# raguilar011095/planet_heightmap_generation

Measured on AMD Instinct MI355X. Metric: Mcells·iter/s, terrain-post erosion stack, higher is better.
Workload: dtype f64

## Files before the change

planet_heightmap_generation_amd/csrc/device.h:

```cpp
#pragma once
#include <hip/hip_runtime.h>

#include <cstdint>
#include <cstdio>
#include <map>
#include <string>
#include <vector>

#include "host_util.h"

#include "erode_ops.h"
#include "flood_ops.h"
#include "wo_internal.h"

namespace wo {

struct HipError { std::string msg; };

#define WO_HIP(call)                                                                                   \
    do {                                                                                               \
        hipError_t e_ = (call);                                                                        \
        if (e_ != hipSuccess)                                                                          \
            throw ::wo::HipError{std::string(#call) + " -> " + hipGetErrorString(e_) + " (" + __FILE__ + ":" + \
                                 std::to_string(__LINE__) + ")"};                                      \
// ... 77 lines not shown
    int32_t* h_count = nullptr;
    float* d_redoE = nullptr; int32_t* d_pendingEver = nullptr; int64_t redoCalls = 0;
    unsigned long long *h_word = nullptr, *d_word = nullptr; uint32_t wordSerial = 0;
    wo::FloodScratch flood;
    wo::FloodExchange floodX;
    void* floodLink = nullptr; void (*floodLinkFree)(void*) = nullptr;
    wo_flood_gpu fgpu;

    int32_t *d_off = nullptr, *d_adj = nullptr;
    float *d_dist = nullptr, *d_xyz = nullptr;
    float *d_e = nullptr, *d_e2 = nullptr, *d_hot = nullptr, *d_orig = nullptr;
    uint8_t *d_ocean = nullptr, *d_coast = nullptr;
    int64_t mirrorMaskVersion = -1;
    uint8_t* d_oceanKnown = nullptr; int32_t* d_maskDiff = nullptr; bool oceanKnownValid = false;
    bool hot_valid = false;
    float* d_savedE = nullptr; uint8_t* d_savedOcean = nullptr; bool saved = false;
    uint8_t* d_tables = nullptr;
    bool scratch = false;
    bool landIdentity = false;
    int64_t floodPrefixMirror = -1, floodPrefixStatic = -1;
    bool floodPrefixOk = false;
    int32_t *d_landIdx = nullptr, *d_land[2] = {nullptr, nullptr}, *d_rank = nullptr;
    int32_t* d_landInit = nullptr; int64_t oceanVersion = 0, landListsOcean = -1; bool landListsMirror = false; int32_t landListsL = -1;
    uint32_t* d_keys[2] = {nullptr, nullptr};
    float *d_cellDist = nullptr, *d_flow = nullptr;
    wo::SolveTask* d_task = nullptr; wo::SolveOut* d_out = nullptr; int32_t *d_haloSend = nullptr, *d_haloRecv = nullptr; float *d_haloBuf = nullptr, *h_haloBuf = nullptr; int32_t nHaloSend = 0, nHaloRecv = 0;
    int32_t* d_flowCnt = nullptr; wo::TargetRank* d_tr = nullptr; wo::EventList* d_ev = nullptr; float* d_me = nullptr;
    int32_t *d_carveSlot = nullptr, *d_carveDeps = nullptr, *d_carveDepCnt = nullptr, *d_carveDepPos = nullptr; uint32_t* d_rs[2] = {nullptr, nullptr}; int rsFlip[2] = {0, 0};    wo::CarveRec* d_carveRecs = nullptr; wo::CarveExpect* d_carveExpect = nullptr; unsigned long long* d_carveG = nullptr;    int32_t* d_carveSlotDone = nullptr; int64_t carveCap = 0;
    unsigned long long* d_accCnt = nullptr;
    int32_t *d_ftLr = nullptr, *d_ftParent = nullptr, *d_ftExtCnt = nullptr; uint32_t* d_ftInflow = nullptr; unsigned long long* d_ftRootAcc = nullptr;
    int32_t *d_jump = nullptr, *d_nj = nullptr;
    int32_t* d_doneAt = nullptr;
    double* d_totalExcess = nullptr;
    float *d_glac = nullptr, *d_iceFlow = nullptr;
    int32_t *d_iceTarget = nullptr, *d_arank = nullptr;
    uint8_t* d_iceUp = nullptr;
    int32_t *d_patchOrder = nullptr, *d_slotOf = nullptr, *d_patchPending = nullptr, *d_patchTotals = nullptr, *d_patchBlk = nullptr; int64_t patchVersion = -1; bool patchMirror = false; int32_t numPatches = 0; int64_t lastPatchLaunches = 1; int64_t solveCalls = 0;
    hipStream_t side = nullptr; hipEvent_t evFork = nullptr, evJoin = nullptr; bool onSide = false;
    uint32_t* d_basinKey = nullptr; int32_t* d_basinVals[2] = {nullptr, nullptr}; int32_t *d_basinJ = nullptr, *d_basinSlot = nullptr, *d_basinRange = nullptr; uint8_t* d_basinLong = nullptr; int64_t basinLaunches = 0; wo::Affine* d_affine[2] = {nullptr, nullptr};    int64_t solvePassSerial = 0;
    int32_t* h_patchTotals = nullptr;
    int32_t *d_listA = nullptr, *d_listB = nullptr, *d_counters = nullptr;
    void* d_sortTemp = nullptr; size_t sortTempBytes = 0;
    int landCur = 0;
    int32_t L = 0;

    struct Import {
        uint8_t* img = nullptr; int64_t imgCap = 0;
        int32_t* label = nullptr;
        uint8_t* flags = nullptr;
        int32_t* lists = nullptr;
        uint8_t* seedOcean = nullptr;
        int32_t* blockCounts = nullptr;
        int32_t* totals = nullptr; int32_t* h_totals = nullptr;
    } imp;

    struct Mirror {
        bool built = false, active = false;
        int32_t *perm = nullptr, *inv = nullptr, *off = nullptr, *adj = nullptr;
        float *dist = nullptr, *xyz = nullptr, *e = nullptr, *e2 = nullptr, *hot = nullptr;
        uint8_t *ocean = nullptr, *coast = nullptr;
        wo::hvec<int32_t> h_perm, h_morton;
        wo::hvec<uint8_t> h_mask;
        int64_t version = 0;
        int32_t *o_off = nullptr, *o_adj = nullptr; float *o_dist = nullptr, *o_xyz = nullptr, *o_e = nullptr, *o_e2 = nullptr;
        uint8_t *o_ocean = nullptr, *o_coast = nullptr;
    } mirror;
// ... 67 lines not shown
```

planet_heightmap_generation_amd/csrc/erode_ops.h:

```cpp
#pragma once
#include <cmath>
#include <cstdint>
#include <cstring>

#include "noise.h"

namespace wo {

constexpr int WO_MAX_DEG = 24;
constexpr int32_t WO_NOT_DONE = 0x7fffffff;

#ifndef WO_TASK_ALIGN
#define WO_TASK_ALIGN 16
#endif
struct alignas(WO_TASK_ALIGN) SolveTask {
    int32_t predSelf, predT, predT2;
    uint32_t flags;
    float e0r, e0t, e0t2;
    float cellDistT;
    double factor;
    int32_t pad_[2];
};
static_assert(sizeof(SolveTask) == 48, "one 48-byte record per task");
#ifndef WO_PATCH_CELLS
// ... 597 lines not shown
        const double h = masked(r);
        int32_t b, nbs[WO_ROW];
        const int deg = load_row(F, r, b, nbs);
        if (deg <= WO_ROW) {
            float mh[WO_ROW], dd[WO_ROW];
#pragma unroll
            for (int k = 0; k < WO_ROW; ++k) mh[k] = masked(nbs[k]);
            load_row_dist(F, b, deg, dd);
#pragma unroll
            for (int k = 0; k < WO_ROW; ++k) {
                const double nh = mh[k];
                if (k >= deg || nh >= h) continue;
                const double d = nd_or_eps(dd[k]);
                if (!talus_may_exceed(h - nh, d, talus)) continue;
                const double slope = (h - nh) / d;
                if (slope > talus) total += (slope - talus) * d;
            }
        } else {
            for (int32_t j = b; j < b + deg; ++j) {
                const double nh = masked(F.adj[j]);
                if (nh >= h) continue;
                const double d = nd_or_eps(F.dist[j]);
                const double slope = (h - nh) / d;
                if (slope > talus) total += (slope - talus) * d;
            }
        }
    }
    F.totalExcess[r] = total;
}

WO_HD inline void thermal_excess_cell(const Fields& F, int32_t r, double talus) { thermal_excess_cell_t(F, r, talus, [&](int32_t c) { return F.me[c]; }); }

template <class Masked>
WO_HD inline float thermal_apply_row(const Fields& F, double h, int32_t myRank, double myTotal, int32_t b, const int32_t (&nbs)[WO_ROW], int deg,
                                     double talus, double kThermal, Masked masked) {
    float mh[WO_ROW], dd[WO_ROW];
#pragma unroll
    for (int k = 0; k < WO_ROW; ++k) mh[k] = masked(nbs[k]);
    load_row_dist(F, b, deg, dd);
    double inSh[WO_ROW], outSh[WO_ROW]; int32_t inRk[WO_ROW]; bool outOn[WO_ROW];
    bool hasOut = false, hasIn = false;
#pragma unroll
    for (int k = 0; k < WO_ROW; ++k) {
        inRk[k] = 0x7fffffff; inSh[k] = 0; outSh[k] = 0; outOn[k] = false;
        const double nh = mh[k], d = nd_or_eps(dd[k]);
        const double gap = fabs(nh - h);
        if (!(k < deg && nh != (double)INFINITY && talus_may_exceed(gap, d, talus))) continue;
        const double slope = gap / d;
        if (!(slope > talus)) continue;
        const bool sends = nh < h;
        if (!sends && !(nh > h)) continue;
        const double tot = sends ? myTotal : F.totalExcess[nbs[k]];
        if (!(tot > 0)) continue;
        const float excess = (float)((slope - talus) * d);
        const double share = ((double)excess / tot) * (kThermal * tot * 0.5);
        if (sends) { hasOut = true; outOn[k] = true; outSh[k] = share; }
        else { hasIn = true; inSh[k] = share; inRk[k] = F.rank[nbs[k]]; }
    }
    if (!hasIn && !hasOut) return (float)(h + 0.0);
    float delta = 0.0f;
    int32_t last = -1;
    bool ownPending = hasOut;
    for (int it = 0; it < WO_ROW + 2; ++it) {
        int32_t pr = 0x7fffffff; double v = 0;
#pragma unroll
        for (int k = 0; k < WO_ROW; ++k) { const bool hit = inRk[k] > last && inRk[k] < pr; pr = hit ? inRk[k] : pr; v = hit ? inSh[k] : v; }
// ... 359 lines not shown
```

planet_heightmap_generation_amd/csrc/flood_kernels.h:

```cpp
#pragma once
#include <hip/hip_runtime.h>

#include "device.h"
#include "flood_ops.h"

namespace wo {

struct FlCtrl {
    int32_t dirtyN[2]; int32_t cur;
    int32_t changedN;
    int32_t pendN[2]; int32_t pcur;
    int32_t release, relIdx;
    int32_t epoch;
    int32_t done;
    int32_t rounds, epochs;
    int32_t overflow;
    int32_t ticket;
    int32_t notFixed, ties;
    int32_t pad_;
    long long evals, changes;
};

struct FlLists { int32_t* dirty[2]; int32_t* pend[2]; int32_t* changed; };

__device__ inline void wave_append(bool flag, int32_t value, int32_t* list, int32_t* counter) {
    const unsigned long long mask = __ballot(flag);
    if (mask == 0) return;
    const int lane = threadIdx.x & 63;
    const int leader = __ffsll((long long)mask) - 1;
    int32_t base = 0;
    if (lane == leader) base = atomicAdd(counter, (int32_t)__popcll(mask));
    base = __shfl(base, leader);
    if (flag) list[base + __popcll(mask & ((1ull << lane) - 1ull))] = value;
}

__global__ __launch_bounds__(WO_BLOCK) void k_fl_init(FloodDev D, float* eL, const float* e, FlCtrl* C) {
    if (blockIdx.x == 0 && threadIdx.x == 0) { FlCtrl z{}; z.epoch = 1; *C = z; }
    WO_GRID_STRIDE(i, D.L) {
        const float v = e[D.cell[i]];
        eL[i] = v;
        FlHead h; h.par = FL_NONE; h.S = v; h.K = 0; h.dep = 0; h.top = 0; h.spare = 0;
        if (D.seedIdx[i] >= 0) {
            h.par = FL_SEED; h.K = (float)((double)v + D.nz[i]); h.dep = 1; h.top = fl_pack(h.K, D.cell[i]);
            D.Astk[(size_t)i * FL_LD] = h.top;
        }
        D.A[i] = h;
        D.fdEpoch[i] = 0; D.inDirty[i] = 0; D.isPending[i] = 0;
    }
}
__global__ __launch_bounds__(WO_BLOCK) void k_fl_seed_dirty(FloodDev D, const int32_t* seeds, int32_t nSeeds, FlLists Ls, FlCtrl* C) {
    WO_BLOCK_STRIDE(s, valid, nSeeds) {
        const int32_t c = valid ? seeds[s] : 0;
        const int32_t b = valid ? D.off[c] : 0, deg = valid ? D.off[c + 1] - b : 0;
        for (int k = 0; __any(k < deg); ++k) {
            bool add = false; int32_t y = -1;
            if (k < deg) { y = D.adj[b + k]; add = D.seedIdx[y] < 0 && atomicExch(&D.inDirty[y], 1) == 0; }
            wave_append(add, y, Ls.dirty[0], &C->dirtyN[0]);
        }
    }
}

__global__ __launch_bounds__(WO_BLOCK) void k_fl_eval(FloodDev D, FlLists Ls, FlCtrl* C) {
    if (C->done) return;
    const bool rel = C->release != 0;
    const int32_t* list = rel ? Ls.pend[C->relIdx] : Ls.dirty[C->cur];
    const int32_t n = rel ? C->pendN[C->relIdx] : C->dirtyN[C->cur];
    const int32_t epoch = C->epoch;
// ... 73 lines not shown
```

planet_heightmap_generation_amd/csrc/kernels_impl.h:

```cpp
#pragma once
#include <hip/hip_runtime.h>
#include <hip/hip_cooperative_groups.h>

#include "device.h"
#include "plates_ops.h"
#include "climate_ops.h"

namespace wo {

#define WO_GRID_STRIDE(i, n) for (int32_t i = blockIdx.x * blockDim.x + threadIdx.x; i < (n); i += gridDim.x * blockDim.x)

#define WO_XCD_CELLS(r, n)                                                                                           \
    for (int32_t xi_ = (int32_t)(blockIdx.x >> 3), xt_ = F.xcdTile,                                                  \
                 r = (int32_t)((((xi_ / xt_) * 8 + (int32_t)(blockIdx.x & 7u)) * xt_ + (xi_ % xt_)) * (int32_t)blockDim.x + (int32_t)threadIdx.x), \
                 once_ = 1;                                                                                          \
         once_ && r < (n); once_ = 0)

#define WO_XCD_LAND(i, r)                                                                                            \
    for (int32_t xi_ = (int32_t)(blockIdx.x >> 3), xt_ = F.xcdTileL,                                                 \
                 i = (int32_t)((((xi_ / xt_) * 8 + (int32_t)(blockIdx.x & 7u)) * xt_ + (xi_ % xt_)) * (int32_t)blockDim.x + (int32_t)threadIdx.x), \
                 once_ = 1;                                                                                          \
         once_ && i < F.L; once_ = 0)                                                                                \
        for (int32_t r = F.landIdx ? F.landIdx[i] : i, once2_ = 1; once2_; once2_ = 0)

#define WO_BLOCK_STRIDE(i, valid, n)                                                              \
    for (int32_t base_ = blockIdx.x * blockDim.x, i = base_ + threadIdx.x, valid = (i < (n));   \
         base_ < (n); base_ += gridDim.x * blockDim.x, i = base_ + threadIdx.x, valid = (i < (n)))

__device__ inline void block_append(bool flag, int32_t value, int32_t* out, int32_t* outCount) {
    __shared__ int32_t s_wave[WO_BLOCK / 64];
    __shared__ int32_t s_base;
    const unsigned long long mask = __ballot(flag);
    const int lane = threadIdx.x & 63, wave = threadIdx.x >> 6;
    const int prefix = __popcll(mask & ((1ull << lane) - 1ull));
    if (lane == 0) s_wave[wave] = __popcll(mask);
    __syncthreads();
    if (threadIdx.x == 0) {
        int32_t tot = 0;
        for (int w = 0; w < WO_BLOCK / 64; ++w) { const int32_t c = s_wave[w]; s_wave[w] = tot; tot += c; }
        s_base = tot ? atomicAdd(outCount, tot) : 0;
    }
    __syncthreads();
    if (flag) out[s_base + s_wave[wave] + prefix] = value;
    __syncthreads();
}

__global__ __launch_bounds__(WO_BLOCK) void k_coast(Fields F, uint8_t* coast) {
    WO_XCD_CELLS(r, F.N) coast[r] = coast_flag(F, r);
}
__global__ __launch_bounds__(WO_BLOCK) void k_ocean_from_elev(const float* e, uint8_t* ocean, int32_t N) {
    WO_GRID_STRIDE(r, N) ocean[r] = (e[r] <= 0.0f) ? 1 : 0;
}
__global__ __launch_bounds__(WO_BLOCK) void k_smooth(Fields F, const float* in, float* out, double strength) {
    WO_XCD_CELLS(r, F.N) out[r] = smooth_cell(F, in, r, strength);
}
__global__ __launch_bounds__(WO_BLOCK) void k_sharpen(Fields F, const float* in, const float* orig, float* out, double strength) {
    WO_XCD_CELLS(r, F.N) out[r] = sharpen_cell(F, in, orig, r, strength);
}
__global__ __launch_bounds__(WO_BLOCK) void k_creep(Fields F, const float* in, float* out, double strength) {
    WO_XCD_CELLS(r, F.N) out[r] = creep_cell(F, in, r, strength);
}
__global__ __launch_bounds__(WO_BLOCK) void k_glacial_blend(Fields F, const float* in, float* out) {
    WO_XCD_CELLS(r, F.N) out[r] = glacial_blend_cell(F, in, r);
}

__device__ inline void load_tables(const uint8_t* tables, uint8_t* sP, uint8_t* sM) {
    for (int i = threadIdx.x; i < 512; i += blockDim.x) { sP[i] = tables[i]; sM[i] = tables[512 + i]; }
    __syncthreads();
}

__global__ __launch_bounds__(WO_BLOCK) void k_noise_eval(const uint8_t* tables, int32_t kind, int32_t octaves, double p0,
                                                          double p1, double p2, int64_t n, const double* xyz, double* out) {
    __shared__ uint8_t sP[512], sM[512];
    load_tables(tables, sP, sM);
    for (int64_t i = blockIdx.x * (int64_t)blockDim.x + threadIdx.x; i < n; i += (int64_t)gridDim.x * blockDim.x) {
        const double x = xyz[3 * i], y = xyz[3 * i + 1], z = xyz[3 * i + 2];
        double v;
// ... 524 lines not shown
        __threadfence_block();
        if (atomicAdd(&s_fin, 1) == aliveWaves - 1) {
            const int32_t done = atomicAdd(&s_done, 0);
            const int32_t left = s_pend - done;
            patchPending[p] = left;
            if (left) atomicAdd(totalPending, left);
            if (dbg) atomicAdd(&dbg[3], done);
        }
    }
}

__global__ __launch_bounds__(WO_BLOCK) void k_solve_blk_init(Fields F, int32_t L) {
    WO_GRID_STRIDE(s, L) {
        if (F.out[s].self.tag != 0) continue;
        const SolveTask T = F.task[s];
        F.blk[s] = T.predT >= 0 ? T.predT : (T.predSelf >= 0 ? T.predSelf : T.predT2);
    }
}
__global__ __launch_bounds__(WO_BLOCK) void k_slot_scatter(const int32_t* patchOrder, int32_t* slotOf, int32_t L) {
    WO_GRID_STRIDE(s, L) slotOf[patchOrder[s]] = s;
}


__global__ __launch_bounds__(WO_BLOCK) void k_solve_final(Fields F, float* out, float* masked) {
    WO_XCD_LAND(i, r) {
        const float v = solve_final_cell(F, r);
        out[r] = v;
        if (masked) masked[r] = v;
    }
}
__global__ __launch_bounds__(WO_BLOCK) void k_fill_i32(int32_t* a, int32_t v, int32_t n) { WO_GRID_STRIDE(i, n) a[i] = v; }

__global__ __launch_bounds__(WO_BLOCK) void k_masked_elev(Fields F) { WO_XCD_LAND(i, r) F.me[r] = F.e[r]; }
__global__ __launch_bounds__(WO_BLOCK) void k_thermal_excess(Fields F, double talus) {
    __shared__ float s_tile[WO_TILE_WIN];
    const TileWindow M = stage_tile(F, F.me, s_tile, WO_XCD_LAND_BASE());
    WO_XCD_LAND(i, r) thermal_excess_cell_t(F, r, talus, M);
}
#ifndef WO_THERMAL_WAVES
#define WO_THERMAL_WAVES 6
#endif
template <int MAXIN>
__global__ __launch_bounds__(WO_BLOCK, WO_THERMAL_WAVES) void k_thermal_apply_reg(Fields F, float* out, double talus, double kThermal) {
    __shared__ float s_tile[WO_TILE_WIN];
    const TileWindow M = stage_tile(F, F.me, s_tile, WO_XCD_LAND_BASE());
    WO_XCD_LAND(i, r) {
        double inShare[MAXIN], outShare[MAXIN]; int32_t inRank[MAXIN];
        out[r] = thermal_apply_cell_t(F, r, talus, kThermal, inShare, inRank, 1, outShare, M);
    }
}
__global__ __launch_bounds__(WO_BLOCK) void k_thermal_apply(Fields F, float* out, double talus, double kThermal, int32_t maxDeg) {
    extern __shared__ __attribute__((aligned(16))) char smem[];
    double* inShare = reinterpret_cast<double*>(smem) + threadIdx.x;
    int32_t* inRank = reinterpret_cast<int32_t*>(smem + (size_t)maxDeg * WO_BLOCK * sizeof(double)) + threadIdx.x;
    WO_XCD_LAND(i, r) out[r] = thermal_apply_cell(F, r, talus, kThermal, inShare, inRank, WO_BLOCK);
}

__global__ __launch_bounds__(WO_BLOCK) void k_glac_index(Fields F, double strength) { WO_XCD_CELLS(r, F.N) F.glac[r] = glac_index_cell(F, r, strength); }
__global__ __launch_bounds__(WO_BLOCK) void k_ice_receivers(Fields F) {
    WO_XCD_CELLS(r, F.N) { ice_receiver_cell(F, r); F.blocker[r] = 0; if (F.ocean[r]) { F.iceFlow[r] = 0.0f; F.iceUp[r] = 0; } }
}
__device__ inline float ld_agent(const float* p) { return __hip_atomic_load(p, __ATOMIC_RELAXED, __HIP_MEMORY_SCOPE_AGENT); }
__device__ inline int32_t ld_agent(const int32_t* p) { return __hip_atomic_load(p, __ATOMIC_RELAXED, __HIP_MEMORY_SCOPE_AGENT); }
__device__ inline void st_agent(float* p, float v) { __hip_atomic_store(p, v, __ATOMIC_RELAXED, __HIP_MEMORY_SCOPE_AGENT); }
__device__ inline void st_agent(int32_t* p, int32_t v) { __hip_atomic_store(p, v, __ATOMIC_RELAXED, __HIP_MEMORY_SCOPE_AGENT); }
__device__ inline void drain_stores() { asm volatile("s_waitcnt vmcnt(0)" ::: "memory"); }

struct IceRow { int32_t nb[WO_ROW]; int32_t rank[WO_ROW]; uint32_t donors; int nd; int deg; };
__device__ inline void ice_row_of(const Fields& F, int32_t t, IceRow& D) {
    int32_t b;
    D.deg = load_row(F, t, b, D.nb);
    D.donors = 0; D.nd = 0;
    if (D.deg > WO_ROW) {
        for (int32_t j = b; j < b + D.deg; ++j) if (F.iceTarget[F.adj[j]] == t) ++D.nd;
        return;
    }
    int32_t tg[WO_ROW];
#pragma unroll
    for (int k = 0; k < WO_ROW; ++k) { tg[k] = F.iceTarget[D.nb[k]]; D.rank[k] = F.rank[D.nb[k]]; }
#pragma unroll
    for (int k = 0; k < WO_ROW; ++k) if (k < D.deg && tg[k] == t) { D.donors |= 1u << k; ++D.nd; }
}
__device__ inline float ice_task_long_row(const Fields& F, int32_t t, int& up) {
    int32_t dn[WO_MAX_DEG]; int nd = 0;
    for (int32_t j = F.off[t]; j < F.off[t + 1]; ++j) { const int32_t n = F.adj[j]; if (F.iceTarget[n] == t) dn[nd++] = n; }
    float acc = F.glac[t];
    int32_t last = -1;
    up = 0;
// ... 287 lines not shown
```

planet_heightmap_generation_amd/csrc/planet.hip:

```cpp
#include <hip/hip_runtime.h>

#include <algorithm>
#include <atomic>
#include <chrono>
#include <cmath>
#include <cstring>

#include "../../include/worogen.h"
#include "device.h"
#include "elevation_host.h"
#include "elevation_kernels.h"
#include "kernels_impl.h"
#include "flood_kernels.h"
#include "elevation_bfs.h"
#include "noise.h"

namespace wo {

const char* const kFamilyNames[FAM_COUNT] = {
    "coast_flags", "smooth_elevation", "sharpen_ridges", "soil_creep", "warp_terrain", "noise_eval", "synthetic_terrain",
    "ocean_from_elevation", "sort_keys", "sort_radix", "rank_scatter", "receivers", "flow_climb",
    "flow_final", "solve_setup", "solve_round", "solve_final", "thermal_excess", "thermal_apply",
    "glac_index", "ice_receivers", "ice_round", "carve_setup", "carve_round", "moraine_fjord", "glacial_blend", "solve_patch", "elev_collisions", "elev_uplift_fused", "plate_grid", "plate_project", "smooth_field", "flood_eval", "flood_apply", "flood_misc", "climate_sweeps", "basin_layout", "basin_sort", "solve_basin", "flow_tiles", "misc", "event_pair_empty", "event_pair_noop_kernel", "event_pair_two_noop_kernels"};

// ... 471 lines not shown
    }
    void resume() {
        if (!on) return;
        auto& M = p->mirror;
        launch(p, FAM_MISC, k_mirror_gather_f32, blocks_for(p->N, 4096), WO_BLOCK, (const float*)M.o_e, (const int32_t*)M.perm, cur, p->N);
        point_at_mirror(cur, cur2);
    }
    void finish() {
        if (!on) return;
        suspend();
        p->mirror.active = on = false;
    }
    ~MirrorScope() { if (on) { point_at_planet(); p->mirror.active = false; } }
};

static void ensure_side_stream(wo_planet* p) {
    if (p->side) return;
    int prLeast = 0, prGreatest = 0;
    WO_HIP(hipDeviceGetStreamPriorityRange(&prLeast, &prGreatest));
    WO_HIP(hipStreamCreateWithPriority(&p->side, hipStreamNonBlocking, prGreatest));
    WO_HIP(hipEventCreateWithFlags(&p->evFork, hipEventDisableTiming)); WO_HIP(hipEventCreateWithFlags(&p->evJoin, hipEventDisableTiming));
}

struct RedoWithChecks {};

struct ErodeCall {
    wo_planet* p;
    int32_t hIters; double K, m, dt; int32_t tIters; double talus, kThermal; int32_t gIters; double gStrength; bool checkEveryPass;
    int32_t total, midIter; double gCarve, gConv, gDep, gFjord;
    int gridN, gridL = 0;
    StageClock clk; MirrorScope mir; FloodRun floodRun;
    int64_t sorts = 0, maxSolve = 0, patchLaunches = 0, basinPasses = 0, basinLeftoverPasses = 0, iceRounds = 0, carveRounds = 0, carveActive = 0, carveFlowLeft = 0;
    double floodHostMs = 0;
    ErodeCall(wo_planet* pl, int32_t h, double K_, double m_, double dt_, int32_t t, double talus_, double kT, int32_t g, double gs, bool check)
        : p(pl), hIters(h), K(K_), m(m_), dt(dt_), tIters(t), talus(talus_), kThermal(kT), gIters(std::max(g, 0)), gStrength(gs != gs ? 0 : gs),
          checkEveryPass(check), total(std::max(hIters, std::max(tIters, gIters))), midIter((int32_t)std::floor(total * 0.75 + 0.5)),
          gridN(xcd_grid(pl->N)), clk(pl), mir(pl) {
        const double gScale = gIters > 0 ? 1.0 / gIters : 0;
        gCarve = 0.02 * gScale; gConv = 0.01 * gScale; gDep = 0.005 * gScale; gFjord = 0.015 * gScale;
    }
    void stats(bool mirrored) const {
        p->erodeStats = {{"land_cells", (double)p->L}, {"mirror_layout", mirrored ? 1.0 : 0.0}, {"iterations", (double)total}, {"sorts", (double)sorts},
                         {"solve_launches_max_per_pass", (double)maxSolve}, {"solve_patch_launches_total", (double)patchLaunches},
                         {"solve_basin_passes", (double)basinPasses}, {"solve_basin_passes_with_leftovers", (double)basinLeftoverPasses},
                         {"flow_two_level", (p->d_ftLr && p->landIdentity && hIters > 0) ? 1.0 : 0.0}, {"ice_rounds_total", (double)iceRounds},
                         {"carve_rounds_total", (double)carveRounds}, {"carve_active_total", (double)carveActive}, {"carve_flow_launches_with_leftovers", (double)carveFlowLeft}, {"solve_check_every_pass", checkEveryPass ? 1.0 : 0.0}, {"calls_run_again_with_checks", (double)p->redoCalls}, {"flood_stage_ms", floodHostMs},
                         {"flood_device_pass1_ms", floodRun.deviceMs}, {"flood_device_rounds", (double)floodRun.rounds}, {"flood_device_epochs", (double)floodRun.epochs},
                         {"flood_device_evaluations", (double)floodRun.evals}, {"flood_equal_key_decisions", (double)floodRun.ties}, {"flood_pass1_on_host", (floodRun.usedDevice && !floodRun.fellBack) ? 0.0 : 1.0},
                         {"flood_host_calls", (double)floodRun.host.calls}, {"flood_host_serial_pass1", (double)floodRun.host.serialPass1}, {"flood_host_tie_groups", (double)floodRun.host.tieGroups}, {"flood_host_contested", (double)floodRun.host.contested},
                         {"flood_host_open_parents", (double)floodRun.host.openParents}, {"flood_host_unresolved", (double)floodRun.host.unresolved},
                         {"flood_host_path_redo", (double)floodRun.host.pathRedo}, {"flood_host_replays", (double)floodRun.host.replays}, {"flood_host_replayed_landmasses", (double)floodRun.host.replayedLandmasses}, {"flood_host_pass1_ms", floodRun.host.pass1Ms},
                         {"flood_host_pass23_ms", floodRun.host.pass23Ms},
                         {"relaxed_sort_every", (double)p->opt.relaxedSortEvery}, {"relaxed_full", p->opt.relaxedFull ? 1.0 : 0.0}, {"flood_exchange_calls", (double)p->floodX.calls}, {"flood_exchange_gathers", (double)p->floodX.gathers}, {"flood_exchange_whole_planet_floods", (double)p->floodX.globalFloods}, {"flood_exchange_received", (double)p->floodX.received}};
    }
};
template <class Cell>
static int32_t compact_land(int64_t n, const uint8_t* ocean, Cell cell, int32_t* out) {
    std::vector<int64_t> cnt(host_threads() + 2, 0);
    parallel_ranges(n, [&](int64_t b, int64_t e, int t) { int64_t c = 0; for (int64_t i = b; i < e; ++i) c += ocean[cell(i)] ? 0 : 1; cnt[t + 1] = c; });
    for (size_t t = 1; t < cnt.size(); ++t) cnt[t] += cnt[t - 1];
    parallel_ranges(n, [&](int64_t b, int64_t e, int t) { int64_t o = cnt[t]; for (int64_t i = b; i < e; ++i) if (!ocean[cell(i)]) out[o++] = (int32_t)i; });
    return (int32_t)cnt.back();
}
static void erode_without_land(ErodeCall& c) {
    wo_planet* p = c.p;
    if (p->floodX.on) {
        hipStream_t s = p->ctx->stream;
        const int calls = (c.hIters > 0 ? 1 : 0) + (c.midIter < c.total ? 1 : 0);
        WO_HIP(hipMemcpyAsync(p->h_pinned, c.mir.on ? p->mirror.o_e : p->d_e, (size_t)p->N * sizeof(float), hipMemcpyDeviceToHost, s));
        WO_HIP(hipStreamSynchronize(s));
        ensure_flood_static(p);
        for (int k = 0; k < calls; ++k) flood_exchange(p, 0.5, nullptr);
    }
    c.mir.finish();
    c.clk.end(); c.clk.finish();
}
static bool erode_setup(ErodeCall& c) {
    wo_planet* p = c.p; hipStream_t s = p->ctx->stream;
    const int32_t N = p->N;
    c.clk.begin("setup");
    refresh_host_ocean(p);
    c.mir.enter(p->h_ocean.data());
    p->landIdentity = c.mir.on && p->mirror.h_mask.size() == (size_t)N;
    coast_flags(p);
    int32_t* hl = reinterpret_cast<int32_t*>(p->h_pinned);
    const uint8_t* oc = p->h_ocean.data();
// ... 203 lines not shown
    }
    const int64_t r = run_solve_patches(p, F, c.K, c.m, c.dt, unchecked, passTag);
    ++c.basinPasses; if (r > 1) ++c.basinLeftoverPasses;
    c.patchLaunches += r; c.maxSolve = std::max(c.maxSolve, r);
    if (!unchecked) launch(p, FAM_SOLVE_FINAL, k_solve_final, c.gridL, WO_BLOCK, F, p->d_e2, (iter < c.tIters) ? p->d_me : (float*)nullptr);
}
static void erode_solve_affine(ErodeCall& c, const Fields& F) {
    wo_planet* p = c.p;
    if (!p->d_affine[0]) { p->d_affine[0] = dalloc<Affine>((size_t)p->N); p->d_affine[1] = dalloc<Affine>((size_t)p->N); }
    launch(p, FAM_SOLVE_SETUP, k_affine_init, c.gridL, WO_BLOCK, F, p->d_affine[0]);
    int cur = 0;
    for (int q = 0; q < 12; ++q, cur ^= 1) launch(p, FAM_SOLVE_ROUND, k_affine_jump, c.gridL, WO_BLOCK, F, (const Affine*)p->d_affine[cur], p->d_affine[cur ^ 1]);
    launch(p, FAM_SOLVE_FINAL, k_affine_apply, c.gridL, WO_BLOCK, F, (const Affine*)p->d_affine[cur], p->d_e2);
}
static void hydraulic_step(ErodeCall& c, int32_t iter) {
    wo_planet* p = c.p;
    Fields F = p->fields();
    F.solveK = c.K; F.solveM = c.m; F.solveDt = c.dt;
    const bool basin = !p->opt.relaxedFull;
    const bool slotIdentity = c.mir.on && p->mirror.h_mask.size() == (size_t)p->N;
    if (basin) { basin_alloc(p); F.basinMslot = slotIdentity ? nullptr : p->d_slotOf; }
    const bool flowTiles = p->landIdentity;
    FlowTiles FT = flowTiles ? flow_tiles_buffers(p) : FlowTiles{};
    const bool tilesBeforeFork = basin && flowTiles && slotIdentity;
    if (tilesBeforeFork) FT.basinJ = p->d_basinJ;
    int32_t* const donorCnt = flowTiles ? (int32_t*)nullptr : p->d_flowCnt;
    erode_receivers(c, F, FT, donorCnt, basin, slotIdentity, tilesBeforeFork);
    erode_flow(c, F, FT, donorCnt, flowTiles, tilesBeforeFork, basin && c.checkEveryPass);
    c.clk.begin("solve");
    if (basin) erode_solve_basin(c, F, iter); else erode_solve_affine(c, F);
    swap_elev(p);
    c.clk.end();
}
static void thermal_step(ErodeCall& c, bool afterSolve) {
    wo_planet* p = c.p;
    c.clk.begin("thermal");
    const Fields F = p->fields();
    if (!afterSolve) launch(p, FAM_THERMAL_EXCESS, k_masked_elev, c.gridL, WO_BLOCK, F);
    launch(p, FAM_THERMAL_EXCESS, k_thermal_excess, c.gridL, WO_BLOCK, F, c.talus);
    if (p->maxDeg <= 12) launch(p, FAM_THERMAL_APPLY, k_thermal_apply_reg<12>, c.gridL, WO_BLOCK, F, p->d_e2, c.talus, c.kThermal);
    else if (p->maxDeg <= 16) launch(p, FAM_THERMAL_APPLY, k_thermal_apply_reg<16>, c.gridL, WO_BLOCK, F, p->d_e2, c.talus, c.kThermal);
    else launch_shmem(p, FAM_THERMAL_APPLY, k_thermal_apply, c.gridL, WO_BLOCK, (size_t)p->maxDeg * WO_BLOCK * 12, F, p->d_e2, c.talus, c.kThermal, (int32_t)p->maxDeg);
    swap_elev(p);
    c.clk.end();
}

static void erode_composite(wo_planet* p, int32_t hIters, double K, double m, double dt, int32_t tIters, double talus,
                            double kThermal, int32_t gIters, double gStrength, bool checkEveryPass = true) {
    ErodeCall c(p, hIters, K, m, dt, tIters, talus, kThermal, gIters, gStrength, checkEveryPass);
    release_stage_brackets(p);
    p->stageTiming.clear(); p->erodeStats.clear();
    p->floodX.calls = 0; p->floodX.gathers = 0; p->floodX.globalFloods = 0; p->floodX.received = 0;
    if (c.total <= 0) return;
    ensure_scratch(p);
    hipStream_t s = p->ctx->stream;
    if (hIters > 0) WO_HIP(hipMemsetAsync(p->d_flowCnt, 0, (size_t)p->N * sizeof(int32_t), s));
    if (hIters > 0 && p->d_ftInflow) { WO_HIP(hipMemsetAsync(p->d_ftInflow, 0, (size_t)p->N * 4, s)); WO_HIP(hipMemsetAsync(p->d_ftExtCnt, 0, (size_t)p->N * 4, s)); }
    if (!erode_setup(c)) return;
    if (hIters > 0) erode_flood(c, 0.5);

    const bool glacial = c.gIters > 0 && c.gStrength > 0;
    if (glacial) launch(p, FAM_GLAC_INDEX, k_glac_index, c.gridN, WO_BLOCK, p->fields(), c.gStrength);
    const bool relaxedFull = p->opt.relaxedFull;
    bool midDone = false, sortAfterFlood = false;
    for (int32_t iter = 0; iter < c.total; ++iter) {
        c.clk.on = true;
        if (!midDone && iter >= c.midIter) { midDone = true; erode_flood(c, 0.85); sortAfterFlood = true; }
        c.clk.on = p->opt.stageTimingAll || p->profiling || c.total <= 16 || iter % 8 == 0;
        const bool gNow = iter < c.gIters && glacial, hNow = iter < hIters;
        const bool sortNow = relaxedFull ? (iter == 0 || sortAfterFlood) : (p->opt.relaxedSortEvery <= 1 || iter % p->opt.relaxedSortEvery == 0);
        if ((gNow || hNow) && sortNow) { sortAfterFlood = false; erode_sort(c); }
        if (gNow) { if (relaxedFull) glacial_step_relaxed(c); else glacial_step_exact(c); }
        if (hNow) {
            if (gNow && sortNow) erode_sort(c);
            hydraulic_step(c, iter);
        }
        if (iter < tIters) thermal_step(c, hNow);
    }
    c.clk.on = true;
    leftovers_so_far(c);
    if (glacial) {
        c.clk.begin("glacial_blend");
        launch(p, FAM_GLAC_BLEND, k_glacial_blend, c.gridN, WO_BLOCK, p->fields(), (const float*)p->d_e, p->d_e2);
        swap_elev(p);
        c.clk.end();
    }
    const bool mirrored = c.mir.on;
    if (mirrored) { c.clk.begin("setup"); c.mir.finish(); c.clk.end(); }
    c.clk.finish();
    c.stats(mirrored);
}

static void jacobi(wo_planet* p, int kind, int32_t iterations, double strength) {
    if (iterations <= 0) return;
    MirrorScope mir(p);
    if (iterations >= 2) mir.enter();
    coast_flags(p);
    const int gridN = xcd_grid(p->N);
    hipStream_t s = p->ctx->stream;
    if (kind == 1) WO_HIP(hipMemcpyAsync(p->d_orig, p->d_e, (size_t)p->N * sizeof(float), hipMemcpyDeviceToDevice, s));
    for (int32_t it = 0; it < iterations; ++it) {
        Fields F = p->fields();
        if (kind == 0) launch(p, FAM_SMOOTH, k_smooth, gridN, WO_BLOCK, F, (const float*)p->d_e, p->d_e2, strength);
        else if (kind == 1) launch(p, FAM_SHARPEN, k_sharpen, gridN, WO_BLOCK, F, (const float*)p->d_e, (const float*)p->d_orig, p->d_e2, strength);
        else launch(p, FAM_CREEP, k_creep, gridN, WO_BLOCK, F, (const float*)p->d_e, p->d_e2, strength);
        swap_elev(p);
    }
    mir.finish();
}

static void upload_tables(wo_planet* p, double seed) {
    uint8_t t[1024];
    noise_tables(seed, t, t + 512);
    WO_HIP(hipMemcpyAsync(p->d_tables, t, 1024, hipMemcpyHostToDevice, p->ctx->stream));
    WO_HIP(hipStreamSynchronize(p->ctx->stream));
}

static void warp(wo_planet* p, double seed, double strength, bool useHot) {
    if (!(strength > 0)) return;
    upload_tables(p, seed + 9999);
    const double maxAmp = 0.12 * strength, bias = 0.25 + 0.5 * strength;
// ... 164 lines not shown
            WO_HIP(hipMemcpyAsync(p->d_dist, nd.data(), (size_t)E * 4, hipMemcpyHostToDevice, s));
            WO_HIP(hipStreamSynchronize(s));
        }
        WO_HIP(hipMemsetAsync(p->d_e, 0, (size_t)N * 4, s));
        WO_HIP(hipMemsetAsync(p->d_ocean, 0, (size_t)N, s));
        WO_HIP(hipEventCreate(&p->evStart)); WO_HIP(hipEventCreate(&p->evStop));
        WO_HIP(hipStreamSynchronize(s));
        return p;
    } catch (const HipError& e) {
        set_error(std::string("wo_planet_create: ") + e.msg);
        if (p) wo_planet_destroy(p);
        return nullptr;
    }
}

void wo_planet_destroy(wo_planet* p) {
    if (!p) return;
    (void)hipSetDevice(p->ctx->device);
    (void)hipStreamSynchronize(p->ctx->stream);
    dfree(p->d_off); dfree(p->d_adj); dfree(p->d_dist); dfree(p->d_xyz); dfree(p->d_e); dfree(p->d_e2); dfree(p->d_hot); dfree(p->d_orig);
    flood_gpu_free(p->fgpu);
    if (p->floodLink && p->floodLinkFree) p->floodLinkFree(p->floodLink);
    p->floodLink = nullptr;
    basin_free(p);
    import_free(p);
    if (p->side) { (void)hipStreamSynchronize(p->side); (void)hipStreamDestroy(p->side); p->side = nullptr; }
    if (p->evFork) { (void)hipEventDestroy(p->evFork); p->evFork = nullptr; }
    if (p->evJoin) { (void)hipEventDestroy(p->evJoin); p->evJoin = nullptr; }
    mirror_free(p);
    dfree(p->d_ocean); dfree(p->d_coast); dfree(p->d_tables); dfree(p->d_savedE); dfree(p->d_savedOcean);
    if (p->d_oceanKnown) { (void)hipFree(p->d_oceanKnown); p->d_oceanKnown = nullptr; } if (p->d_maskDiff) { (void)hipFree(p->d_maskDiff); p->d_maskDiff = nullptr; }
    dfree(p->d_landInit); dfree(p->d_landIdx); dfree(p->d_land[0]); dfree(p->d_land[1]); dfree(p->d_keys[0]); dfree(p->d_keys[1]); dfree(p->d_rank);
    dfree(p->d_cellDist); dfree(p->d_flow); dfree(p->d_task); dfree(p->d_out); dfree(p->d_flowCnt); dfree(p->d_tr); dfree(p->d_ev); dfree(p->d_me); dfree(p->d_haloSend); dfree(p->d_haloRecv); dfree(p->d_haloBuf); if (p->h_haloBuf) { (void)hipHostFree(p->h_haloBuf); p->h_haloBuf = nullptr; } dfree(p->d_carveSlot); dfree(p->d_redoE); dfree(p->d_pendingEver); for (auto& r : p->d_rs) { if (r) (void)hipFree(r); r = nullptr; } dfree(p->d_carveG); dfree(p->d_carveExpect); dfree(p->d_carveRecs); dfree(p->d_carveSlotDone); dfree(p->d_carveDeps); dfree(p->d_carveDepCnt); dfree(p->d_carveDepPos); dfree(p->d_ftLr); dfree(p->d_ftParent); dfree(p->d_affine[0]); dfree(p->d_affine[1]); dfree(p->d_ftExtCnt); dfree(p->d_ftInflow); dfree(p->d_ftRootAcc); dfree(p->d_accCnt); dfree(p->d_jump); dfree(p->d_nj);
    dfree(p->d_doneAt); dfree(p->d_totalExcess);
    dfree(p->d_glac); dfree(p->d_iceFlow); dfree(p->d_iceTarget); dfree(p->d_arank); dfree(p->d_iceUp);
    dfree(p->d_patchOrder); dfree(p->d_slotOf); dfree(p->d_patchPending); dfree(p->d_patchTotals); dfree(p->d_patchBlk);
    dfree(p->d_listA); dfree(p->d_listB); dfree(p->d_counters);
    if (p->h_patchTotals) (void)hipHostFree(p->h_patchTotals);
    if (p->d_sortTemp) (void)hipFree(p->d_sortTemp);
    if (p->h_pinned) (void)hipHostFree(p->h_pinned);
    if (p->h_count) (void)hipHostFree(p->h_count);
    if (p->h_word) { (void)hipHostFree(p->h_word); p->h_word = nullptr; }
    for (auto& pe : p->pending) { (void)hipEventDestroy(pe.a); (void)hipEventDestroy(pe.b); }
    for (auto& b : p->stageBrackets) { (void)hipEventDestroy(b.a); (void)hipEventDestroy(b.b); }
    for (auto e : p->eventPool) (void)hipEventDestroy(e);
    if (p->evStart) (void)hipEventDestroy(p->evStart);
    if (p->evStop) (void)hipEventDestroy(p->evStop);
    delete p;
}

int wo_planet_upload(wo_planet* p, const float* r_elevation, const uint8_t* r_isOcean) {
    if (!check_planet(p, "wo_planet_upload")) return 1;
    WO_TRY
    hipStream_t s = p->ctx->stream;
    if (r_elevation) WO_HIP(hipMemcpyAsync(p->d_e, r_elevation, (size_t)p->N * 4, hipMemcpyHostToDevice, s));
    if (r_isOcean) {
        WO_HIP(hipMemcpyAsync(p->d_ocean, r_isOcean, (size_t)p->N, hipMemcpyHostToDevice, s));
        if (p->h_ocean.size() != (size_t)p->N || std::memcmp(p->h_ocean.data(), r_isOcean, (size_t)p->N) != 0) {
            p->h_ocean.assign(r_isOcean, r_isOcean + p->N);
            p->flood.staticValid = false; ++p->oceanVersion;
            p->oceanKnownValid = false;
        }
        p->h_ocean_valid = true;
    }
    WO_HIP(hipStreamSynchronize(s));
    return 0;
    WO_CATCH("wo_planet_upload")
// ... 675 lines not shown
```

Measured before the change: 6311.

## Compact thermal apply to cells with over-talus slopes via sharded worklist

The thermal excess kernel now detects whether any neighbour slope exceeds talus. Untouched cells get their elevation copied straight to the output, and touched cells are appended to a sharded per-iteration list using wave-level ballot atomics. The apply kernels then process only the listed cells instead of every land cell. This drops the shared-memory tile staging in apply and adds per-call counters plus a host sync at the end to gather statistics. The risks are atomic contention, scattered access in the compacted apply, and the added synchronization.

Measured after the change: 6330 (median of 4 runs). About the same (+0.3%).

```diff
diff --git a/planet_heightmap_generation_amd/csrc/device.h b/planet_heightmap_generation_amd/csrc/device.h
--- a/planet_heightmap_generation_amd/csrc/device.h
+++ b/planet_heightmap_generation_amd/csrc/device.h
@@ -133,6 +133,7 @@
     int32_t *d_jump = nullptr, *d_nj = nullptr;
     int32_t* d_doneAt = nullptr;
     double* d_totalExcess = nullptr;
+    int32_t *d_thermalList = nullptr, *d_thermalCnt = nullptr; int64_t thermalListCap = 0; int32_t thermalCntIters = 0;
     float *d_glac = nullptr, *d_iceFlow = nullptr;
     int32_t *d_iceTarget = nullptr, *d_arank = nullptr;
     uint8_t* d_iceUp = nullptr;
diff --git a/planet_heightmap_generation_amd/csrc/erode_ops.h b/planet_heightmap_generation_amd/csrc/erode_ops.h
--- a/planet_heightmap_generation_amd/csrc/erode_ops.h
+++ b/planet_heightmap_generation_amd/csrc/erode_ops.h
@@ -653,6 +653,46 @@
 WO_HD inline void thermal_excess_cell(const Fields& F, int32_t r, double talus) { thermal_excess_cell_t(F, r, talus, [&](int32_t c) { return F.me[c]; }); }
 
 template <class Masked>
+WO_HD inline bool thermal_detect_cell_t(const Fields& F, int32_t r, double talus, float* out, Masked masked) {
+    if (F.ocean[r]) return false;
+    const double h = masked(r);
+    double total = 0;
+    bool touched = false;
+    int32_t b, nbs[WO_ROW];
+    const int deg = load_row(F, r, b, nbs);
+    if (deg <= WO_ROW) {
+        float mh[WO_ROW], dd[WO_ROW];
+#pragma unroll
+        for (int k = 0; k < WO_ROW; ++k) mh[k] = masked(nbs[k]);
+        load_row_dist(F, b, deg, dd);
+#pragma unroll
+        for (int k = 0; k < WO_ROW; ++k) {
+            const double nh = mh[k];
+            if (k >= deg || nh == h || nh == (double)INFINITY) continue;
+            const double d = nd_or_eps(dd[k]);
+            const double gap = fabs(nh - h);
+            if (!talus_may_exceed(gap, d, talus)) continue;
+            const double slope = gap / d;
+            if (!(slope > talus)) continue;
+            touched = true;
+            if (nh < h) total += (slope - talus) * d;
+        }
+    } else {
+        for (int32_t j = b; j < b + deg; ++j) {
+            const double nh = masked(F.adj[j]);
+            if (nh == h || nh == (double)INFINITY) continue;
+            const double d = nd_or_eps(F.dist[j]);
+            const double slope = fabs(nh - h) / d;
+            if (!(slope > talus)) continue;
+            touched = true;
+            if (nh < h) total += (slope - talus) * d;
+        }
+    }
+    if (touched) F.totalExcess[r] = total; else out[r] = (float)(h + 0.0);
+    return touched;
+}
+
+template <class Masked>
 WO_HD inline float thermal_apply_row(const Fields& F, double h, int32_t myRank, double myTotal, int32_t b, const int32_t (&nbs)[WO_ROW], int deg,
                                      double talus, double kThermal, Masked masked) {
     float mh[WO_ROW], dd[WO_ROW];
diff --git a/planet_heightmap_generation_amd/csrc/flood_kernels.h b/planet_heightmap_generation_amd/csrc/flood_kernels.h
--- a/planet_heightmap_generation_amd/csrc/flood_kernels.h
+++ b/planet_heightmap_generation_amd/csrc/flood_kernels.h
@@ -22,17 +22,6 @@
 };
 
 struct FlLists { int32_t* dirty[2]; int32_t* pend[2]; int32_t* changed; };
-
-__device__ inline void wave_append(bool flag, int32_t value, int32_t* list, int32_t* counter) {
-    const unsigned long long mask = __ballot(flag);
-    if (mask == 0) return;
-    const int lane = threadIdx.x & 63;
-    const int leader = __ffsll((long long)mask) - 1;
-    int32_t base = 0;
-    if (lane == leader) base = atomicAdd(counter, (int32_t)__popcll(mask));
-    base = __shfl(base, leader);
-    if (flag) list[base + __popcll(mask & ((1ull << lane) - 1ull))] = value;
-}
 
 __global__ __launch_bounds__(WO_BLOCK) void k_fl_init(FloodDev D, float* eL, const float* e, FlCtrl* C) {
     if (blockIdx.x == 0 && threadIdx.x == 0) { FlCtrl z{}; z.epoch = 1; *C = z; }
diff --git a/planet_heightmap_generation_amd/csrc/kernels_impl.h b/planet_heightmap_generation_amd/csrc/kernels_impl.h
--- a/planet_heightmap_generation_amd/csrc/kernels_impl.h
+++ b/planet_heightmap_generation_amd/csrc/kernels_impl.h
@@ -43,6 +43,16 @@
     __syncthreads();
     if (flag) out[s_base + s_wave[wave] + prefix] = value;
     __syncthreads();
+}
+
+__device__ inline void wave_append(bool flag, int32_t value, int32_t* out, int32_t* outCount) {
+    const unsigned long long mask = __ballot(flag);
+    if (mask == 0) return;
+    const int lane = threadIdx.x & 63, leader = __ffsll((long long)mask) - 1;
+    int32_t base = 0;
+    if (lane == leader) base = atomicAdd(outCount, (int32_t)__popcll(mask));
+    base = __shfl(base, leader);
+    if (flag) out[base + __popcll(mask & ((1ull << lane) - 1ull))] = value;
 }
 
 __global__ __launch_bounds__(WO_BLOCK) void k_coast(Fields F, uint8_t* coast) {
@@ -633,28 +643,45 @@
 __global__ __launch_bounds__(WO_BLOCK) void k_fill_i32(int32_t* a, int32_t v, int32_t n) { WO_GRID_STRIDE(i, n) a[i] = v; }
 
 __global__ __launch_bounds__(WO_BLOCK) void k_masked_elev(Fields F) { WO_XCD_LAND(i, r) F.me[r] = F.e[r]; }
-__global__ __launch_bounds__(WO_BLOCK) void k_thermal_excess(Fields F, double talus) {
+constexpr int WO_THERMAL_SHARDS = 64;
+constexpr int WO_THERMAL_CNT_STRIDE = 32;
+struct ThermalList { int32_t* cells; int32_t* count; int32_t cap; };
+__device__ inline int32_t thermal_listed_cell(const ThermalList& T) {
+    const int32_t s = (int32_t)(blockIdx.x % WO_THERMAL_SHARDS), i = (int32_t)((blockIdx.x / WO_THERMAL_SHARDS) * blockDim.x + threadIdx.x);
+    return i < T.count[s * WO_THERMAL_CNT_STRIDE] ? T.cells[(size_t)s * T.cap + i] : -1;
+}
+__global__ __launch_bounds__(WO_BLOCK) void k_thermal_excess(Fields F, double talus, float* out, ThermalList T) {
     __shared__ float s_tile[WO_TILE_WIN];
     const TileWindow M = stage_tile(F, F.me, s_tile, WO_XCD_LAND_BASE());
-    WO_XCD_LAND(i, r) thermal_excess_cell_t(F, r, talus, M);
+    bool touched = false; int32_t cell = 0;
+    WO_XCD_LAND(i, r) { cell = r; touched = thermal_detect_cell_t(F, r, talus, out, M); }
+    const int32_t s = (int32_t)(blockIdx.x % WO_THERMAL_SHARDS);
+    wave_append(touched, cell, T.cells + (size_t)s * T.cap, T.count + s * WO_THERMAL_CNT_STRIDE);
+}
+__global__ __launch_bounds__(WO_BLOCK) void k_thermal_list_totals(const int32_t* counts, int32_t iters, int32_t* totals) {
+    WO_GRID_STRIDE(i, iters) {
+        int32_t n = 0;
+        for (int s = 0; s < WO_THERMAL_SHARDS; ++s) n += counts[((size_t)i * WO_THERMAL_SHARDS + s) * WO_THERMAL_CNT_STRIDE];
+        totals[i] = n;
+    }
 }
 #ifndef WO_THERMAL_WAVES
 #define WO_THERMAL_WAVES 6
 #endif
 template <int MAXIN>
-__global__ __launch_bounds__(WO_BLOCK, WO_THERMAL_WAVES) void k_thermal_apply_reg(Fields F, float* out, double talus, double kThermal) {
-    __shared__ float s_tile[WO_TILE_WIN];
-    const TileWindow M = stage_tile(F, F.me, s_tile, WO_XCD_LAND_BASE());
-    WO_XCD_LAND(i, r) {
-        double inShare[MAXIN], outShare[MAXIN]; int32_t inRank[MAXIN];
-        out[r] = thermal_apply_cell_t(F, r, talus, kThermal, inShare, inRank, 1, outShare, M);
-    }
-}
-__global__ __launch_bounds__(WO_BLOCK) void k_thermal_apply(Fields F, float* out, double talus, double kThermal, int32_t maxDeg) {
+__global__ __launch_bounds__(WO_BLOCK, WO_THERMAL_WAVES) void k_thermal_apply_reg(Fields F, float* out, double talus, double kThermal, ThermalList T) {
+    const int32_t c = thermal_listed_cell(T);
+    if (c < 0) return;
+    double inShare[MAXIN], outShare[MAXIN]; int32_t inRank[MAXIN];
+    out[c] = thermal_apply_cell(F, c, talus, kThermal, inShare, inRank, 1, outShare);
+}
+__global__ __launch_bounds__(WO_BLOCK) void k_thermal_apply(Fields F, float* out, double talus, double kThermal, int32_t maxDeg, ThermalList T) {
     extern __shared__ __attribute__((aligned(16))) char smem[];
     double* inShare = reinterpret_cast<double*>(smem) + threadIdx.x;
     int32_t* inRank = reinterpret_cast<int32_t*>(smem + (size_t)maxDeg * WO_BLOCK * sizeof(double)) + threadIdx.x;
-    WO_XCD_LAND(i, r) out[r] = thermal_apply_cell(F, r, talus, kThermal, inShare, inRank, WO_BLOCK);
+    const int32_t c = thermal_listed_cell(T);
+    if (c < 0) return;
+    out[c] = thermal_apply_cell(F, c, talus, kThermal, inShare, inRank, WO_BLOCK);
 }
 
 __global__ __launch_bounds__(WO_BLOCK) void k_glac_index(Fields F, double strength) { WO_XCD_CELLS(r, F.N) F.glac[r] = glac_index_cell(F, r, strength); }
diff --git a/planet_heightmap_generation_amd/csrc/planet.hip b/planet_heightmap_generation_amd/csrc/planet.hip
--- a/planet_heightmap_generation_amd/csrc/planet.hip
+++ b/planet_heightmap_generation_amd/csrc/planet.hip
@@ -527,6 +527,7 @@
     StageClock clk; MirrorScope mir; FloodRun floodRun;
     int64_t sorts = 0, maxSolve = 0, patchLaunches = 0, basinPasses = 0, basinLeftoverPasses = 0, iceRounds = 0, carveRounds = 0, carveActive = 0, carveFlowLeft = 0;
     double floodHostMs = 0;
+    int32_t thermalIters = 0; int64_t thermalListed = 0, thermalListedLast = 0;
     ErodeCall(wo_planet* pl, int32_t h, double K_, double m_, double dt_, int32_t t, double talus_, double kT, int32_t g, double gs, bool check)
         : p(pl), hIters(h), K(K_), m(m_), dt(dt_), tIters(t), talus(talus_), kThermal(kT), gIters(std::max(g, 0)), gStrength(gs != gs ? 0 : gs),
           checkEveryPass(check), total(std::max(hIters, std::max(tIters, gIters))), midIter((int32_t)std::floor(total * 0.75 + 0.5)),
@@ -546,7 +547,8 @@
                          {"flood_host_open_parents", (double)floodRun.host.openParents}, {"flood_host_unresolved", (double)floodRun.host.unresolved},
                          {"flood_host_path_redo", (double)floodRun.host.pathRedo}, {"flood_host_replays", (double)floodRun.host.replays}, {"flood_host_replayed_landmasses", (double)floodRun.host.replayedLandmasses}, {"flood_host_pass1_ms", floodRun.host.pass1Ms},
                          {"flood_host_pass23_ms", floodRun.host.pass23Ms},
-                         {"relaxed_sort_every", (double)p->opt.relaxedSortEvery}, {"relaxed_full", p->opt.relaxedFull ? 1.0 : 0.0}, {"flood_exchange_calls", (double)p->floodX.calls}, {"flood_exchange_gathers", (double)p->floodX.gathers}, {"flood_exchange_whole_planet_floods", (double)p->floodX.globalFloods}, {"flood_exchange_received", (double)p->floodX.received}};
+                         {"relaxed_sort_every", (double)p->opt.relaxedSortEvery}, {"relaxed_full", p->opt.relaxedFull ? 1.0 : 0.0}, {"flood_exchange_calls", (double)p->floodX.calls}, {"flood_exchange_gathers", (double)p->floodX.gathers}, {"flood_exchange_whole_planet_floods", (double)p->floodX.globalFloods}, {"flood_exchange_received", (double)p->floodX.received},
+                         {"thermal_listed_cells_total", (double)thermalListed}, {"thermal_listed_cells_last", (double)thermalListedLast}};
     }
 };
 template <class Cell>
@@ -816,15 +818,49 @@
     swap_elev(p);
     c.clk.end();
 }
+static void thermal_list_begin(wo_planet* p, int32_t tIters) {
+    if (tIters > p->thermalCntIters) {
+        dfree(p->d_thermalCnt);
+        p->thermalCntIters = tIters + tIters / 2;
+        p->d_thermalCnt = dalloc<int32_t>((size_t)p->thermalCntIters * (WO_THERMAL_SHARDS * WO_THERMAL_CNT_STRIDE + 1));
+    }
+    WO_HIP(hipMemsetAsync(p->d_thermalCnt, 0, (size_t)tIters * WO_THERMAL_SHARDS * WO_THERMAL_CNT_STRIDE * sizeof(int32_t), p->ctx->stream));
+}
+static ThermalList thermal_list(ErodeCall& c, int32_t iter) {
+    wo_planet* p = c.p;
+    ThermalList T;
+    T.cap = ((c.gridL + WO_THERMAL_SHARDS - 1) / WO_THERMAL_SHARDS) * WO_BLOCK;
+    const int64_t need = (int64_t)T.cap * WO_THERMAL_SHARDS;
+    if (need > p->thermalListCap) {
+        dfree(p->d_thermalList);
+        p->d_thermalList = dalloc<int32_t>((size_t)need);
+        p->thermalListCap = need;
+    }
+    T.cells = p->d_thermalList;
+    T.count = p->d_thermalCnt + (size_t)iter * WO_THERMAL_SHARDS * WO_THERMAL_CNT_STRIDE;
+    return T;
+}
+static void thermal_list_end(ErodeCall& c) {
+    wo_planet* p = c.p; hipStream_t s = p->ctx->stream;
+    if (c.thermalIters <= 0) return;
+    int32_t* totals = p->d_thermalCnt + (size_t)p->thermalCntIters * WO_THERMAL_SHARDS * WO_THERMAL_CNT_STRIDE;
+    launch(p, FAM_MISC, k_thermal_list_totals, blocks_for(c.thermalIters), WO_BLOCK, (const int32_t*)p->d_thermalCnt, c.thermalIters, totals);
+    std::vector<int32_t> h((size_t)c.thermalIters);
+    WO_HIP(hipMemcpyAsync(h.data(), totals, h.size() * sizeof(int32_t), hipMemcpyDeviceToHost, s));
+    WO_HIP(hipStreamSynchronize(s));
+    for (int32_t n : h) c.thermalListed += n;
+    c.thermalListedLast = h.back();
+}
 static void thermal_step(ErodeCall& c, bool afterSolve) {
     wo_planet* p = c.p;
     c.clk.begin("thermal");
     const Fields F = p->fields();
+    const ThermalList T = thermal_list(c, c.thermalIters++);
     if (!afterSolve) launch(p, FAM_THERMAL_EXCESS, k_masked_elev, c.gridL, WO_BLOCK, F);
-    launch(p, FAM_THERMAL_EXCESS, k_thermal_excess, c.gridL, WO_BLOCK, F, c.talus);
-    if (p->maxDeg <= 12) launch(p, FAM_THERMAL_APPLY, k_thermal_apply_reg<12>, c.gridL, WO_BLOCK, F, p->d_e2, c.talus, c.kThermal);
-    else if (p->maxDeg <= 16) launch(p, FAM_THERMAL_APPLY, k_thermal_apply_reg<16>, c.gridL, WO_BLOCK, F, p->d_e2, c.talus, c.kThermal);
-    else launch_shmem(p, FAM_THERMAL_APPLY, k_thermal_apply, c.gridL, WO_BLOCK, (size_t)p->maxDeg * WO_BLOCK * 12, F, p->d_e2, c.talus, c.kThermal, (int32_t)p->maxDeg);
+    launch(p, FAM_THERMAL_EXCESS, k_thermal_excess, c.gridL, WO_BLOCK, F, c.talus, p->d_e2, T);
+    if (p->maxDeg <= 12) launch(p, FAM_THERMAL_APPLY, k_thermal_apply_reg<12>, c.gridL, WO_BLOCK, F, p->d_e2, c.talus, c.kThermal, T);
+    else if (p->maxDeg <= 16) launch(p, FAM_THERMAL_APPLY, k_thermal_apply_reg<16>, c.gridL, WO_BLOCK, F, p->d_e2, c.talus, c.kThermal, T);
+    else launch_shmem(p, FAM_THERMAL_APPLY, k_thermal_apply, c.gridL, WO_BLOCK, (size_t)p->maxDeg * WO_BLOCK * 12, F, p->d_e2, c.talus, c.kThermal, (int32_t)p->maxDeg, T);
     swap_elev(p);
     c.clk.end();
 }
@@ -840,6 +876,7 @@
     hipStream_t s = p->ctx->stream;
     if (hIters > 0) WO_HIP(hipMemsetAsync(p->d_flowCnt, 0, (size_t)p->N * sizeof(int32_t), s));
     if (hIters > 0 && p->d_ftInflow) { WO_HIP(hipMemsetAsync(p->d_ftInflow, 0, (size_t)p->N * 4, s)); WO_HIP(hipMemsetAsync(p->d_ftExtCnt, 0, (size_t)p->N * 4, s)); }
+    if (tIters > 0) thermal_list_begin(p, tIters);
     if (!erode_setup(c)) return;
     if (hIters > 0) erode_flood(c, 0.5);
 
@@ -871,6 +908,7 @@
     }
     const bool mirrored = c.mir.on;
     if (mirrored) { c.clk.begin("setup"); c.mir.finish(); c.clk.end(); }
+    thermal_list_end(c);
     c.clk.finish();
     c.stats(mirrored);
 }
@@ -1101,7 +1139,7 @@
     if (p->d_oceanKnown) { (void)hipFree(p->d_oceanKnown); p->d_oceanKnown = nullptr; } if (p->d_maskDiff) { (void)hipFree(p->d_maskDiff); p->d_maskDiff = nullptr; }
     dfree(p->d_landInit); dfree(p->d_landIdx); dfree(p->d_land[0]); dfree(p->d_land[1]); dfree(p->d_keys[0]); dfree(p->d_keys[1]); dfree(p->d_rank);
     dfree(p->d_cellDist); dfree(p->d_flow); dfree(p->d_task); dfree(p->d_out); dfree(p->d_flowCnt); dfree(p->d_tr); dfree(p->d_ev); dfree(p->d_me); dfree(p->d_haloSend); dfree(p->d_haloRecv); dfree(p->d_haloBuf); if (p->h_haloBuf) { (void)hipHostFree(p->h_haloBuf); p->h_haloBuf = nullptr; } dfree(p->d_carveSlot); dfree(p->d_redoE); dfree(p->d_pendingEver); for (auto& r : p->d_rs) { if (r) (void)hipFree(r); r = nullptr; } dfree(p->d_carveG); dfree(p->d_carveExpect); dfree(p->d_carveRecs); dfree(p->d_carveSlotDone); dfree(p->d_carveDeps); dfree(p->d_carveDepCnt); dfree(p->d_carveDepPos); dfree(p->d_ftLr); dfree(p->d_ftParent); dfree(p->d_affine[0]); dfree(p->d_affine[1]); dfree(p->d_ftExtCnt); dfree(p->d_ftInflow); dfree(p->d_ftRootAcc); dfree(p->d_accCnt); dfree(p->d_jump); dfree(p->d_nj);
-    dfree(p->d_doneAt); dfree(p->d_totalExcess);
+    dfree(p->d_doneAt); dfree(p->d_totalExcess); dfree(p->d_thermalList); dfree(p->d_thermalCnt);
     dfree(p->d_glac); dfree(p->d_iceFlow); dfree(p->d_iceTarget); dfree(p->d_arank); dfree(p->d_iceUp);
     dfree(p->d_patchOrder); dfree(p->d_slotOf); dfree(p->d_patchPending); dfree(p->d_patchTotals); dfree(p->d_patchBlk);
     dfree(p->d_listA); dfree(p->d_listB); dfree(p->d_counters);
```
